# liaoherui/StrainScan

Hardware: AMD Instinct MI355X
Metric: M reads/sec vs 1433-strain E. coli DB (higher is better)
Workload: dtype u64

## Files before the change

### strainscan_amd/csrc/ss_mini.hip

```cpp
#include "ss_common.h"
#include "ss_scan_dev.h"

#include <algorithm>
#include <atomic>
#include <mutex>
#include <type_traits>


namespace {

using namespace ss::dev;

constexpr int MT = 64;
static_assert(MT == 64, "one wave per workgroup: phase 2 compacts with ballots and keeps its counters in scalar registers");
#ifndef SS_Q1CAP
#define SS_Q1CAP 160
#endif
constexpr int Q1CAP = SS_Q1CAP;
static_assert(Q1CAP <= 4096, "q2 keeps a q1b index in 12 bits");
constexpr int Q1CAP_RT = 256;
constexpr int NUM_SGPR = 80;
constexpr int RPL = 2;
constexpr int RPL2 = 1;
constexpr int U3 = 4;
constexpr int MLANES = MT - 2;
constexpr int MTILE = MLANES * PPT;

template <int CAP>
struct QSharedT {
    uint32_t code_[MT + 3];
    uint16_t inv[MT + 2];
    uint32_t q1[CAP + 64];
    alignas(16) uint8_t ib[MT * PPT];
    uint64_t q2[CAP];
    uint32_t cnt[4];
};
template <int CAP>
struct QBloomT {
    uint64_t q1b[CAP];
};

constexpr int COMB_NE = 64;
constexpr int COMB_CH = 4;
constexpr uint32_t COMB_NONE = 0xFFu;
template <int CAP>
struct QCombT {
    static_assert(CAP <= 256, "run indices in bytes");
    uint32_t key[COMB_NE];
    uint32_t nrun[COMB_NE];
    uint32_t acc[COMB_NE][5];
    uint8_t ent[CAP];
    uint8_t list[COMB_NE];
    uint8_t rest[CAP];
};

template <class QS>
__device__ __forceinline__ void kmer_at(const QS &S, uint32_t pos, uint32_t &lo, uint32_t &hi, uint32_t khi_mask = 0x3FFFFFFFu)
{
    const uint32_t w = pos >> 4, sh = 2 * (pos & 15);
    const uint32_t a = S.code_[w + 1], b = S.code_[w + 2], c = S.code_[w + 3];
    lo = __builtin_amdgcn_alignbit(b, a, sh);
    hi = __builtin_amdgcn_alignbit(c, b, sh) & khi_mask;
}

template <class QS>
__device__ __forceinline__ uint32_t mmer_at(const QS &S, uint32_t p)
{
    const uint32_t w = p >> 4;
    return __builtin_amdgcn_alignbit(S.code_[w + 2], S.code_[w + 1], 2 * (p & 15)) & ss::M30;
}
template <class QS>
__device__ __forceinline__ uint32_t win16_at(const QS &S, int32_t p)
{
    const int32_t w = (p >> 4) + 1;
    return __builtin_amdgcn_alignbit(S.code_[w + 1], S.code_[w], 2 * (p & 15));
}

__device__ __forceinline__ uint32_t cand_slot(uint32_t bstart, uint32_t amask, uint32_t q, uint32_t F = 16u)
{
    const uint32_t o = F - q;
    return ((amask >> o) & 1u) ? bstart + 1u + (uint32_t)__popc(amask & ((1u << o) - 1u)) : 0u;
}
__device__ __forceinline__ uint32_t aligned_mask(uint32_t hdr, uint32_t o0, uint32_t F = 16u)
{
    const uint32_t wm = (2u << F) - 1u;
    return ((hdr & wm) << (F - o0)) & wm;
}

template <bool COMB>
__device__ __forceinline__ void count_slot(uint32_t cpos, uint32_t bstart, uint32_t ent, uint32_t *__restrict__ acc5,
                                           uint32_t *__restrict__ counts)
{
    const uint32_t off = cpos - bstart;
    if (COMB && ent != COMB_NONE && off < 20u) atomicAdd(&acc5[ent * 5u + (off >> 2)], 1u << ((off & 3u) * 8u));
    else atomicAdd(&counts[cpos], 1u);
}
template <bool COMB, class QS>
__device__ __forceinline__ void settle_item(const QS &S, uint32_t pos, uint32_t bstart, uint32_t multi, uint32_t cpos,
                                            uint64_t cand, const uint64_t *__restrict__ mkeys,
                                            uint32_t *__restrict__ counts, uint32_t ent = COMB_NONE, uint32_t *__restrict__ acc5 = nullptr,
                                            uint32_t khi_mask = 0x3FFFFFFFu)
{
    uint32_t klo, khi;
    kmer_at(S, pos, klo, khi, khi_mask);
    if ((uint32_t)cand == klo && (uint32_t)(cand >> 32) == khi) {
        count_slot<COMB>(cpos, bstart, ent, acc5, counts);
    } else if (multi) {
        const uint64_t km = ((uint64_t)khi << 32) | klo;
        const uint32_t cnt = (uint32_t)(mkeys[bstart] >> 32);
        for (uint32_t q = 0; q < cnt; q++)
            if (mkeys[bstart + 1 + q] == km) { count_slot<COMB>(bstart + 1 + q, bstart, ent, acc5, counts); break; }
    }
}

__device__ __forceinline__ uint32_t mad24s(uint32_t a, uint32_t b, uint32_t c)
{
    uint32_t d;
    asm("v_mad_u32_u24 %0, %1, %2, %3" : "=v"(d) : "v"(a), "v"(b), "s"(c));
    return d;
}
#define SS_MIN_DPP(i, j) "v_min_u32_dpp %" #i ", %" #j ", %" #i " wave_shl:1 row_mask:0xf bank_mask:0xf bound_ctrl:1\n\t"
__device__ __forceinline__ void min_next_lane8(uint32_t &a0, uint32_t &a1, uint32_t &a2, uint32_t &a3, uint32_t &a4, uint32_t &a5,
                                               uint32_t &a6, uint32_t &a7, uint32_t p0, uint32_t p1, uint32_t p2, uint32_t p3,
                                               uint32_t p4, uint32_t p5, uint32_t p6, uint32_t p7)
{
    asm("s_nop 1\n\t" SS_MIN_DPP(0, 8) SS_MIN_DPP(1, 9) SS_MIN_DPP(2, 10) SS_MIN_DPP(3, 11) SS_MIN_DPP(4, 12) SS_MIN_DPP(5, 13)
        SS_MIN_DPP(6, 14) SS_MIN_DPP(7, 15)
        : "+v"(a0), "+v"(a1), "+v"(a2), "+v"(a3), "+v"(a4), "+v"(a5), "+v"(a6), "+v"(a7)
        : "v"(p0), "v"(p1), "v"(p2), "v"(p3), "v"(p4), "v"(p5), "v"(p6), "v"(p7));
}
__device__ __forceinline__ uint32_t shift_in_ne(uint32_t m, uint32_t a, uint32_t b)
{
    asm("v_cmp_ne_u32 vcc, %1, %2\n\tv_addc_co_u32 %0, vcc, %0, %0, vcc" : "+v"(m) : "v"(a), "v"(b) : "vcc");
    return m;
}

__device__ uint32_t ss_probe_runs[64];

#define SS_MARK(i) asm volatile("; SSMARK " #i)

constexpr int MULTI_MAX = 4;
struct ScanTabs {
    const uint64_t *mkeys[MULTI_MAX];
    const uint4 *pages[MULTI_MAX];
    uint32_t *counts[MULTI_MAX];
    const uint32_t *bloom[MULTI_MAX];
    uint32_t n_pages[MULTI_MAX], cbase[MULTI_MAX], bloom_shift[MULTI_MAX];
    int n;
};

template <int W>
__device__ __forceinline__ void sliding_min(const uint32_t (&x)[32], uint32_t (&out)[PPT])
{
    constexpr int P = W >= 16 ? 16 : W >= 8 ? 8 : W >= 4 ? 4 : 2;
    uint32_t m[32];
#pragma unroll
    for (int i = 0; i < 32; i++) m[i] = x[i];
#pragma unroll
    for (int s2 = 1; s2 < P; s2 <<= 1) {
#pragma unroll
        for (int i = 0; i + s2 < 32; i++) m[i] = min(m[i], m[i + s2]);
    }
#pragma unroll
    for (int j = 0; j < PPT; j++) out[j] = min(m[j], m[j + W - P]);
}

template <int IN, bool BLOOM, bool COMB, int WAVES_PER_SIMD, bool MULTI = false, int KK = 31>
__global__ __launch_bounds__(MT, WAVES_PER_SIMD) __attribute__((amdgpu_num_sgpr(NUM_SGPR))) void scan_mini_kernel(
    const uint8_t *__restrict__ bases, uint64_t n, uint64_t n_tiles, const uint64_t *__restrict__ mkeys0,
    const uint4 *__restrict__ pages0, uint32_t n_pages0, uint32_t *__restrict__ counts0, uint32_t cbase0,
    const uint32_t *__restrict__ bloom, uint32_t bloom_shift, uint32_t xcd_swizzle, const ScanTabs tabs, int k_rt)
{
    static_assert(!(COMB && BLOOM), "a combining scan is for tables that expect hits: they have no use for the minimizer filter");
    static_assert(KK == 31 || KK == 0, "k = 31, or k at run time");
    const uint64_t *__restrict__ mkeys = mkeys0;
    const uint4 *__restrict__ pages = pages0;
    uint32_t *__restrict__ counts = counts0;
    uint32_t n_pages = n_pages0, cbase = cbase0, tab_key = 0u;
    const int K = KK ? KK : k_rt;
    const uint32_t W = (uint32_t)(K - ss::MINI_M + 1), F = W - 1u;
    const uint32_t khi_mask = (1u << (2 * K - 32)) - 1u;
    const uint32_t fmask = F >= 16u ? 0xFFFFFFFFu : (1u << (2u * F)) - 1u;
    static_assert(31 - ss::MINI_M + 1 == PPT + 1, "k = 31: a k-mer window = own m-mers j..15 + neighbour m-mers 0..j");
    constexpr int QC = KK == 31 ? Q1CAP : Q1CAP_RT;
    __shared__ QSharedT<QC> S;
    __shared__ QBloomT<QC> SB;
    __shared__ QCombT<QC> C;
    const int t = threadIdx.x;
    const uint32_t vc1 = ss::MMK_C1;
    constexpr uint64_t CH = COMB ? COMB_CH : 1;

    uint64_t tile = (uint64_t)blockIdx.x * CH, tile_end = n_tiles, stride = gridDim.x, tile0 = 0;
    if (xcd_swizzle & 1u) {
        const uint64_t per = (((n_tiles + 7) >> 3) + CH - 1) / CH * CH, x = blockIdx.x & 7u;
        stride = gridDim.x >> 3;
        tile0 = x * per;
        tile = tile0 + (uint64_t)(blockIdx.x >> 3) * CH;
        tile_end = min(n_tiles, (x + 1) * per);
    }
    auto next_tile = [&](uint64_t tl) -> uint64_t {
        if (CH == 1) return tl + stride;
        return ((tl + 1 - tile0) % CH) ? tl + 1 : tl + 1 + (stride - 1) * CH;
    };
    uint32_t comb_runs = 0;
    if (COMB) {
        C.key[t] = 0u;
        C.nrun[t] = 0u;
#pragma unroll
        for (int w = 0; w < 5; w++) C.acc[t][w] = 0u;
    }
    auto comb_flush = [&]() {
        const uint32_t key = C.key[t];
        const uint64_t occ = __ballot(key != 0u);
        const uint32_t nocc = (uint32_t)__popcll(occ);
        if (key) C.list[__builtin_amdgcn_mbcnt_hi((uint32_t)(occ >> 32), __builtin_amdgcn_mbcnt_lo((uint32_t)occ, 0u))] = (uint8_t)t;
        __syncthreads();
        for (uint32_t g0 = 0; g0 < nocc * 16u; g0 += MT) {
            const uint32_t g = g0 + (uint32_t)t;
            if ((g >> 4) < nocc) {
                const uint32_t e = C.list[g >> 4], off = 1u + (g & 15u);
                const uint32_t c = (C.acc[e][off >> 2] >> ((off & 3u) * 8u)) & 0xFFu;
                if (c) {
                    const uint32_t k1 = C.key[e] - 1u;
                    uint32_t *cb = MULTI ? tabs.counts[k1 >> 30] : counts;
                    atomicAdd(&cb[(k1 & ss::START_MASK) + off], c);
                }
            }
        }
        if (key) {
            const uint32_t w = C.acc[t][4] >> 8;
            if (w) {
                uint32_t *cb = MULTI ? tabs.counts[(key - 1u) >> 30] : counts;
#pragma unroll
                for (uint32_t o = 0; o < 3; o++)
                    if ((w >> (8u * o)) & 0xFFu) atomicAdd(&cb[((key - 1u) & ss::START_MASK) + 17u + o], (w >> (8u * o)) & 0xFFu);
            }
        }
        __syncthreads();
        if (key) {
            C.key[t] = 0u;
            C.nrun[t] = 0u;
#pragma unroll
            for (int w = 0; w < 5; w++) C.acc[t][w] = 0u;
        }
        __syncthreads();
        comb_runs = 0;
    };
    uint32_t wn[4];
    if (tile < tile_end) {
        const uint64_t b0 = tile * MTILE;
        load_in<IN>(bases, b0 + (uint64_t)t * 16, n, wn);
    }
    for (; tile < tile_end; tile = next_tile(tile)) {
        SS_MARK(20);
        {
            uint32_t code, inv;
            decode_in<IN>(wn, code, inv);
            S.code_[t + 1] = code;
            S.inv[t] = (uint16_t)inv;
            if (t == 1) S.cnt[1] = 0;
            const uint64_t nt = next_tile(tile);
            if (nt < tile_end) {
                const uint64_t nb = nt * (uint64_t)MTILE;
                load_in<IN>(bases, nb + (uint64_t)t * 16, n, wn);
            }
        }
        __syncthreads();
        SS_MARK(0);

        uint32_t hm[PPT];
        {
            const uint32_t c0 = S.code_[t + 1], c1 = S.code_[t + 2];
            hm[0] = mad24s(c0, vc1, ss::MMK_C0);
#pragma unroll
            for (int i = 1; i < PPT; i++) hm[i] = mad24s(__builtin_amdgcn_alignbit(c1, c0, 2 * i), vc1, ss::MMK_C0 + (uint32_t)i);
        }
        SS_MARK(1);

        uint32_t live = 0;
        if (KK == 31 && t < MLANES) {
            uint32_t lo;
            __builtin_memcpy(&lo, &S.inv[t], 4);
            uint32_t hi = __builtin_amdgcn_alignbit(S.inv[t + 2], lo, 31);
            lo = __builtin_bitreverse32(lo & 0x7FFFFFFFu);
            lo |= lo << 1; lo |= lo << 2; lo |= lo << 4; lo |= lo << 8; lo |= lo << 16;
            hi |= hi << 1; hi |= hi << 2; hi |= hi << 4; hi |= hi << 8;
            live = ~(__builtin_bitreverse32(lo) | (hi << 1)) & 0xFFFFu;
        } else if (KK != 31 && t < MLANES) {
            uint64_t y = (uint64_t)S.inv[t] | ((uint64_t)S.inv[t + 1] << 16) | ((uint64_t)S.inv[t + 2] << 32);
            y |= y >> 1; y |= y >> 2; y |= y >> 4; y |= y >> 8;
            y |= y >> (K - 16);
            live = ~(uint32_t)y & 0xFFFFu;
        }
        uint32_t need = 0;
        uint32_t mh[PPT];
        if (KK == 31) {
            uint32_t pf[PPT];
            pf[0] = hm[0] + 16u;
#pragma unroll
            for (int j = 1; j < PPT; j++) pf[j] = min(pf[j - 1], hm[j] + 16u);
#pragma unroll
            for (int i = PPT - 2; i >= 0; i--) hm[i] = min(hm[i], hm[i + 1]);
            min_next_lane8(hm[0], hm[1], hm[2], hm[3], hm[4], hm[5], hm[6], hm[7], pf[0], pf[1], pf[2], pf[3], pf[4], pf[5], pf[6], pf[7]);
            min_next_lane8(hm[8], hm[9], hm[10], hm[11], hm[12], hm[13], hm[14], hm[15], pf[8], pf[9], pf[10], pf[11], pf[12], pf[13], pf[14], pf[15]);
#pragma unroll
            for (int j = 0; j < PPT; j++) mh[j] = hm[j];
        } else {
            uint32_t x[32];
#pragma unroll
            for (int i = 0; i < PPT; i++) {
                x[i] = hm[i];
                x[PPT + i] = (uint32_t)__builtin_amdgcn_update_dpp(0, (int)hm[i], 0x130, 0xf, 0xf, false) + 16u;
            }
            switch (W) {
            case 3: sliding_min<3>(x, mh); break;   case 4: sliding_min<4>(x, mh); break;   case 5: sliding_min<5>(x, mh); break;
            case 6: sliding_min<6>(x, mh); break;   case 7: sliding_min<7>(x, mh); break;   case 8: sliding_min<8>(x, mh); break;
            case 9: sliding_min<9>(x, mh); break;   case 10: sliding_min<10>(x, mh); break; case 11: sliding_min<11>(x, mh); break;
            case 12: sliding_min<12>(x, mh); break; case 13: sliding_min<13>(x, mh); break; case 14: sliding_min<14>(x, mh); break;
            case 15: sliding_min<15>(x, mh); break; default: sliding_min<16>(x, mh); break;
            }
        }
        if (live) {
            uint32_t chg = 0u;
#pragma unroll
            for (int j = PPT - 1; j >= 1; j--) chg = shift_in_ne(chg, mh[j], mh[j - 1]);
            chg = (chg << 1) | 1u;
            need = live & (chg | (~live << 1));
            uint32_t pk[4];
#pragma unroll
            for (int w = 0; w < 4; w++) {
                const uint32_t lo = __builtin_amdgcn_perm(mh[4 * w + 1], mh[4 * w], 0x0c0c0400u);
                const uint32_t hi = __builtin_amdgcn_perm(mh[4 * w + 3], mh[4 * w + 2], 0x0c0c0400u);
                pk[w] = __builtin_amdgcn_perm(hi, lo, 0x05040100u);
            }
            reinterpret_cast<uint4 *>(S.ib)[t] = make_uint4(pk[0], pk[1], pk[2], pk[3]);
        }
        SS_MARK(6);
        const uint32_t stop = need | (~live & 0xFFFFu) | 0x10000u;
        uint32_t ext12 = 0;
        {
            const uint32_t first = (uint32_t)__ffs(stop >> 1);
            const uint32_t ownlast = (live >> 15) ? (uint32_t)__clz(need) - 15u : 0u;
            const uint32_t l_mh = (uint32_t)__builtin_amdgcn_update_dpp(0, (int)mh[PPT - 1], 0x138, 0xf, 0xf, false);
            const uint32_t l_own = (uint32_t)__builtin_amdgcn_update_dpp(0, (int)ownlast, 0x138, 0xf, 0xf, false);
            const bool cont = (live & 1u) && l_own && l_mh == mh[0] + 16u && l_own + first <= 16u;
            const uint32_t give = cont ? first << 12 : 0u;
            ext12 = (uint32_t)__builtin_amdgcn_update_dpp(0, (int)give, 0x130, 0xf, 0xf, false);
            if (cont) need &= ~1u;
        }
        uint32_t ovf = 0;
        uint32_t n1;
        {
            const uint32_t mine = (uint32_t)__popc(need);
            const uint32_t incl = wave_inclusive_sum(mine);
            n1 = min((uint32_t)__builtin_amdgcn_readlane((int)incl, 63), (uint32_t)QC);
            const uint32_t mybase = incl - mine;
            if (need) {
                const uint32_t dummy = (uint32_t)QC + (uint32_t)t;
                const uint32_t stop1 = stop >> 1, tbase = (uint32_t)(t * PPT);
                uint32_t idx = mybase;
                for (uint32_t nd = need; nd; idx++) {
                    const uint32_t j = (uint32_t)__ffs(nd) - 1u;
                    nd &= nd - 1u;
                    const uint32_t len = (uint32_t)__ffs(stop1 >> j);
                    S.q1[min(idx, dummy)] = (len << 12) + (tbase + j + (nd ? 0u : ext12));
                }
                if (mybase + mine > (uint32_t)QC) {
                    uint32_t r = mybase;
                    for (uint32_t nd = need; nd; nd &= nd - 1u, r++)
                        if (r >= (uint32_t)QC) ovf |= nd & (0u - nd);
                }
            }
        }
        __syncthreads();
        SS_MARK(2);

        auto run_meta = [&](uint32_t e) {
            const uint32_t rpos = e & 0xFFFu;
            return e | ((((uint32_t)S.ib[rpos] & 31u) - (rpos & 15u)) << 17);
        };
        auto push_found = [&](uint32_t lo, uint32_t mask17, uint32_t meta, uint32_t ridx, bool queued) {
            const uint32_t bstart = lo & ss::START_MASK, multi = lo >> 31;
            const uint32_t amask = aligned_mask(mask17, (meta >> 17) & 31u, F);
            uint32_t i2 = QC;
            if (queued) i2 = atomicAdd(&S.cnt[1], 1u);
            if (i2 < QC) {
                S.q2[i2] = ((uint64_t)(lo & (ss::START_MASK | ss::PG_SOLID)) << 32) | (multi << 31) | (amask << 12) | ridx;
            } else {
                const uint32_t rpos = meta & 0xFFFu, len = (meta >> 12) & 31u;
                for (uint32_t q = 0; q < len; q++) {
                    const uint32_t cpos = cand_slot(bstart, amask, q, F);
                    if (cpos) settle_item<false>(S, rpos + q, bstart, multi, cpos, mkeys[cpos], mkeys, counts, COMB_NONE, nullptr, khi_mask);
                }
            }
        };
        auto scan_page = [&](const uint4 tg, uint32_t page, uint32_t meta, uint32_t h, uint32_t ridx, bool queued) -> bool {
            const uint32_t tt = (h & 0xFFu) * 0x01010101u;
            const uint32_t x0 = tg.x ^ tt, x1 = tg.y ^ tt;
            const uint32_t z0 = ~(((x0 & 0x7F7F7F7Fu) + 0x7F7F7F7Fu) | x0) & 0x80808080u;
            const uint32_t z1 = ~(((x1 & 0x7F7F7F7Fu) + 0x7F7F7F7Fu) | x1) & 0x80808080u;
            uint32_t hit = (z0 >> 7) | (z1 >> 3);
            if (hit) {
                const uint32_t o0 = (meta >> 17) & 31u, len = (meta >> 12) & 31u;
                const char *pb = reinterpret_cast<const char *>(pages) + (uint64_t)page * 64u;
                do {
                    const uint32_t b = (uint32_t)__ffs(hit) - 1u, sl = (b >> 3) + (b & 4u);
                    hit &= hit - 1u;
                    const uint32_t hi8 = (((b & 4u) ? tg.w : tg.z) >> (b & 24u)) & 0xFFu;
                    const bool ref = hi8 & 0x80u;
                    const uint32_t e = hi8 & 31u, j = o0 + e - F;
                    if (ref ? ((hi8 ^ (h >> 8)) & 0x3Fu) == 0u : j < len) {
                        const uint32_t lo = reinterpret_cast<const uint32_t *>(pb + 16)[sl];
                        const uint32_t mid = reinterpret_cast<const uint16_t *>(pb + 48)[sl];
                        if (ref) {
                            push_found(lo, mid | ((hi8 & 0x40u) << 10), meta, ridx, queued);
                        } else if ((mid >> 4) == ((h >> 8) & 0xFFFu)) {
                            const int32_t q = (int32_t)((meta & 0xFFFu) + o0);
                            const uint32_t fa = win16_at(S, q + ss::MINI_M), fb = win16_at(S, q - (int32_t)F);
                            const uint32_t m = ((1u << e) << e) - 1u;
                            if ((((fa & m) | (fb & ~m)) & fmask) == lo) atomicAdd(&counts[cbase + page * 8u + sl], 1u);
                        }
                    }
                } while (hit);
            }
            return (tg.w >> 24) != (uint32_t)ss::PG_EMPTY_HI;
        };
        auto scan_more = [&](uint32_t page, uint32_t meta, uint32_t h, uint32_t ridx, bool queued) {
            uint4 tg;
            do {
                page++;
                tg = pages[(uint64_t)page * 4u];
            } while (scan_page(tg, page, meta, h, ridx, queued));
        };

        SS_MARK(7);
        for (int tb = 0; tb < (MULTI ? tabs.n : 1); tb++) {
        if (MULTI) {
            mkeys = tabs.mkeys[tb]; pages = tabs.pages[tb]; counts = tabs.counts[tb];
            n_pages = tabs.n_pages[tb]; cbase = tabs.cbase[tb]; tab_key = (uint32_t)tb << 30;
            if (BLOOM) { bloom = tabs.bloom[tb]; bloom_shift = tabs.bloom_shift[tb]; }
            if (tb) {
                if (t == 1) S.cnt[1] = 0;
                __syncthreads();
            }
        }
        uint32_t ns = n1;
        if (BLOOM) {
            ns = 0;
            for (uint32_t r0 = 0; r0 < n1; r0 += RPL * MT) {
                SS_MARK(11);
                uint32_t meta[RPL], hs[RPL], bw[RPL];
                bool ok[RPL];
#pragma unroll
                for (int u = 0; u < RPL; u++) {
                    const uint32_t r = r0 + u * MT + t;
                    ok[u] = r < n1;
                    meta[u] = run_meta(S.q1[ok[u] ? r : 0u]);
                    hs[u] = ss::mix30(mmer_at(S, (meta[u] & 0xFFFu) + (meta[u] >> 17)));
                }
#pragma unroll
                for (int u = 0; u < RPL; u++) bw[u] = bloom[hs[u] >> (bloom_shift + 5)];
#pragma unroll
                for (int u = 0; u < RPL; u++) ok[u] = ok[u] && ((bw[u] >> ((hs[u] >> bloom_shift) & 31u)) & 1u);
#pragma unroll
                for (int u = 0; u < RPL; u++) {
                    const uint64_t pass = __ballot(ok[u]);
                    if (ok[u]) SB.q1b[ns + __builtin_amdgcn_mbcnt_hi((uint32_t)(pass >> 32), __builtin_amdgcn_mbcnt_lo((uint32_t)pass, 0u))] =
                        ((uint64_t)hs[u] << 32) | meta[u];
                    ns += (uint32_t)__popcll(pass);
                }
            }
            __syncthreads();
        }
        for (uint32_t i0 = 0; i0 < ns; i0 += RPL2 * MT) {
            SS_MARK(12);
            uint32_t meta[RPL2], hs[RPL2], pgi[RPL2];
            uint4 tg[RPL2];
            bool ok[RPL2];
#pragma unroll
            for (int u = 0; u < RPL2; u++) {
                const uint32_t i = i0 + u * MT + t;
                ok[u] = i < ns;
                if (BLOOM) {
                    const uint64_t sv = SB.q1b[ok[u] ? i : 0u];
                    meta[u] = (uint32_t)sv;
                    hs[u] = (uint32_t)(sv >> 32);
                } else {
                    meta[u] = run_meta(S.q1[ok[u] ? i : 0u]);
                    hs[u] = ss::mix30(mmer_at(S, (meta[u] & 0xFFFu) + (meta[u] >> 17)));
                }
                pgi[u] = ss::page_of(hs[u], n_pages);
                if (ok[u]) tg[u] = pages[(uint64_t)pgi[u] * 4u];
            }
            SS_MARK(13);
#pragma unroll
            for (int u = 0; u < RPL2; u++)
                if (ok[u] && scan_page(tg[u], pgi[u], meta[u], hs[u], i0 + u * MT + t, true)) scan_more(pgi[u], meta[u], hs[u], i0 + u * MT + t, true);
            SS_MARK(14);
        }
        __syncthreads();
        SS_MARK(3);

        {
            const uint32_t n2 = min(S.cnt[1], (uint32_t)QC);
            if (!COMB && (xcd_swizzle & 2u) && t == 0) atomicAdd(&ss_probe_runs[blockIdx.x & 63u], n2);
            bool comb_full = false;
            if (COMB) {
                SS_MARK(10);
                comb_runs += n2;
                for (uint32_t r = (uint32_t)t; r < n2; r += MT) {
                    const uint32_t key = (((uint32_t)(S.q2[r] >> 32) & ss::START_MASK) | tab_key) + 1u;
                    uint32_t i = (key * 0x9E3779B1u) >> 26, e = COMB_NONE;
                    static_assert(COMB_NE == 64, "hash: top six bits");
                    for (int pr = 0; pr < 8; pr++) {
                        const uint32_t old = atomicCAS(&C.key[i], 0u, key);
                        if (old == 0u || old == key) { e = atomicAdd(&C.nrun[i], 1u) < 255u ? i : COMB_NONE; break; }
                        i = (i + 1u) & (COMB_NE - 1u);
                    }
                    C.ent[r] = (uint8_t)e;
                    comb_full = comb_full || e == COMB_NONE;
                }
                comb_full = __ballot(comb_full) != 0ull;
                __syncthreads();
                SS_MARK(9);
            }
            uint32_t n_rest = 0, n_hit = 0;
            auto cand_round = [&](auto UC, uint32_t g0) {
                constexpr int U = decltype(UC)::value;
                SS_MARK(15);
                uint32_t pos[U], bst[U], mul[U], cps[U], ent[U];
                uint64_t cnd[U];
#pragma unroll
                for (int u = 0; u < U; u++) {
                    const uint32_t g = g0 + u * MT + t, q = g & 15u;
                    const bool v = (g >> 4) < n_rest;
                    const uint32_t fi = v ? (COMB ? (uint32_t)C.rest[g >> 4] : (g >> 4)) : 0u;
                    const uint64_t r = S.q2[fi];
                    const uint32_t run = BLOOM ? (uint32_t)SB.q1b[(uint32_t)r & 0xFFFu] : S.q1[(uint32_t)r & 0xFFFu];
                    pos[u] = (run & 0xFFFu) + q;
                    bst[u] = (uint32_t)(r >> 32) & ss::START_MASK;
                    mul[u] = (uint32_t)r >> 31;
                    cps[u] = (v && q < ((run >> 12) & 31u)) ? cand_slot(bst[u], ((uint32_t)r >> 12) & 0x1FFFFu, q, F) : 0u;
                    cnd[u] = mkeys[cps[u]];
                    ent[u] = COMB ? (uint32_t)C.ent[fi] : COMB_NONE;
                }
#pragma unroll
                for (int u = 0; u < U; u++)
                    if (cps[u]) settle_item<COMB>(S, pos[u], bst[u], mul[u], cps[u], cnd[u], mkeys, counts, ent[u], &C.acc[0][0], khi_mask);
                SS_MARK(16);
            };
            if (!COMB) n_rest = n2;
            for (uint32_t r0 = 0; COMB && r0 < n2; r0 += MT) {
                const uint32_t r = r0 + (uint32_t)t;
                const bool v = r < n2;
                const uint64_t q = S.q2[v ? r : 0u];
                const bool solid = v && ((q >> 62) & 1ull);
                uint32_t hitmask = 0;
                const uint64_t om = __ballot(v && !solid);
                if (v && !solid) C.rest[n_rest + __builtin_amdgcn_mbcnt_hi((uint32_t)(om >> 32), __builtin_amdgcn_mbcnt_lo((uint32_t)om, 0u))] = (uint8_t)r;
                n_rest += (uint32_t)__popcll(om);
                if (solid) {
                    const uint32_t bstart = (uint32_t)(q >> 32) & ss::START_MASK, amask = ((uint32_t)q >> 12) & 0x1FFFFu;
                    const uint32_t run = BLOOM ? (uint32_t)SB.q1b[(uint32_t)q & 0xFFFu] : S.q1[(uint32_t)q & 0xFFFu];
                    const uint32_t rpos = run & 0xFFFu, len = (run >> 12) & 31u;
                    const uint32_t am = amask & ~((1u << (W - len)) - 1u);
                    if (am) {
                        const uint32_t o_hi = 31u - (uint32_t)__clz(am), o_lo = (uint32_t)__ffs(am) - 1u, d = o_hi - o_lo;
                        const uint32_t slot_a = bstart + 1u + (uint32_t)__popc(amask & ((1u << o_hi) - 1u));
                        const uint64_t k1 = mkeys[slot_a], k2 = mkeys[slot_a - d];
                        const int32_t P = (int32_t)(rpos + F - o_hi);
                        const uint64_t lo64 = k1 | (k2 << (2u * d));
                        const uint32_t hi32 = d ? (uint32_t)(k2 >> (64u - 2u * d)) : 0u;
                        uint32_t x0 = win16_at(S, P) ^ (uint32_t)lo64;
                        const uint32_t nb1 = d + (uint32_t)K - 16u, nb2 = d + (uint32_t)K > 32u ? d + (uint32_t)K - 32u : 0u;
                        uint32_t x1 = (win16_at(S, P + 16) ^ (uint32_t)(lo64 >> 32)) & (nb1 >= 16u ? 0xFFFFFFFFu : (1u << (2u * nb1)) - 1u);
                        uint32_t x2 = nb2 ? (win16_at(S, P + 32) ^ hi32) & ((1u << (2u * nb2)) - 1u) : 0u;
                        uint32_t match = (2u << d) - 1u;
                        x0 = (x0 | (x0 >> 1)) & 0x55555555u; x1 = (x1 | (x1 >> 1)) & 0x55555555u; x2 = (x2 | (x2 >> 1)) & 0x55555555u;
                        auto strike = [&](uint32_t xb, uint32_t base0) {
                            while (xb) {
                                const uint32_t m = base0 + (((uint32_t)__ffs(xb) - 1u) >> 1);
                                xb &= xb - 1u;
                                const uint32_t hi = min(m, d), lw = m > (uint32_t)K - 1u ? m - ((uint32_t)K - 1u) : 0u;
                                if (lw <= hi) match &= ~(((2u << hi) - 1u) & ~((1u << lw) - 1u));
                            }
                        };
                        strike(x0, 0u); strike(x1, 16u); strike(x2, 32u);
                        if (match) {
                            const uint32_t w_ = 1u;
                            const uint32_t off_a = slot_a - bstart;
                            const uint32_t e_ = COMB ? (uint32_t)C.ent[r] : COMB_NONE;
                            if (COMB && e_ != COMB_NONE && off_a < 20u) {
                                const uint32_t bits = __brev(match) >> (31u - off_a);
#pragma unroll
                                for (uint32_t wd = 0; wd < 5; wd++) {
                                    const uint32_t nib = (bits >> (4u * wd)) & 15u;
                                    if (nib) atomicAdd(&C.acc[e_][wd], ((nib * 0x00204081u) & 0x01010101u) * w_);
                                }
                            } else {
                                hitmask = match;
                                S.q2[r] = ((uint64_t)slot_a << 32) | match;
                            }
                        }
                    }
                }
                const uint64_t hm = __ballot(hitmask != 0u);
                if (hitmask) C.rest[QC - 1u - (n_hit + __builtin_amdgcn_mbcnt_hi((uint32_t)(hm >> 32), __builtin_amdgcn_mbcnt_lo((uint32_t)hm, 0u)))] = (uint8_t)r;
                n_hit += (uint32_t)__popcll(hm);
            }
            if (COMB) __syncthreads();
            for (uint32_t g0 = 0; g0 < n_hit * 16u; g0 += MT) {
                const uint32_t g = g0 + (uint32_t)t;
                if ((g >> 4) < n_hit) {
                    const uint64_t e = S.q2[C.rest[QC - 1u - (g >> 4)]];
                    const uint32_t j = g & 15u, slot_a = (uint32_t)(e >> 32), mt = (uint32_t)e;
                    if ((mt >> j) & 1u) atomicAdd(&counts[slot_a - j], 1u);
                    if (j == 0u && (mt >> 16)) atomicAdd(&counts[slot_a - 16u], 1u);
                }
            }
            const uint32_t total = n_rest * 16u;
            uint32_t g0 = 0;
            for (; g0 < total; g0 += U3 * MT) cand_round(std::integral_constant<int, U3>(), g0);
            if (COMB && comb_full) { __syncthreads(); SS_MARK(4); comb_flush(); SS_MARK(8); }
        }
        if (ovf) {
            for (int j = 0; j < PPT; j++) {
                if (!((ovf >> j) & 1u)) continue;
                const uint32_t len12 = ((uint32_t)__ffs(stop >> (j + 1)) << 12) + ((need >> (j + 1)) ? 0u : ext12);
                const uint32_t meta = run_meta(len12 + (uint32_t)(t * PPT + j));
                const uint32_t h = ss::mix30(mmer_at(S, (meta & 0xFFFu) + (meta >> 17)));
                const uint32_t page = ss::page_of(h, n_pages);
                if (scan_page(pages[(uint64_t)page * 4u], page, meta, h, 0u, false)) scan_more(page, meta, h, 0u, false);
            }
        }
        if (MULTI && tb + 1 < tabs.n) __syncthreads();
        }
        SS_MARK(4);
        __syncthreads();
        SS_MARK(5);
        if (COMB && CH > 1 && comb_runs && ((tile + 1 - tile0) % CH) == 0) { comb_flush(); SS_MARK(8); }
    }
    if (COMB && comb_runs) comb_flush();
}

}

namespace ss {

std::atomic<long long> g_hook_generic_k{0};

constexpr uint64_t PROBE_TILES = 8192;
constexpr double PROBE_RUNS_PER_TILE = 8.0;
static std::mutex probe_mu;

static bool probe_known(ss_db *db, uint64_t set_id, bool *comb)
{
    std::lock_guard<std::mutex> g(probe_mu);
    if (db->probe_set != set_id) return false;
    *comb = db->probe_comb != 0;
    return true;
}

static bool choose_comb(bool flagged, bool binned, bool several, int k, bool verdict)
{
    static const int env = [] { const char *e = getenv("SS_COMBINE"); return e ? atoi(e) : -1; }();
    if (several) return flagged && (env < 0 ? binned : env != 0);
    if (k != 31 || env < 0) return binned && (flagged || (k == 31 && verdict));
    return env == 2 ? binned : (flagged && env != 0);
}

constexpr int scan_mini_waves(bool comb, int kk) { return kk == 0 ? 5 : (comb ? 6 : 8); }

static int launch_scan_mini_pass(ss_db *const *dbs, int n_dbs, bool several, bool bloom, bool comb, bool probe, const uint8_t *b,
                                 uint64_t n, bool packed, hipStream_t stream)
{
    const int k = dbs[0]->k;
    if ((bloom && comb) || (bloom && several && k != 31)) return SS_EINVAL;
    ScanTabs tabs = {};
    for (int i = 0; i < n_dbs; i++) {
        const ss_db *db = dbs[i];
        tabs.mkeys[i] = db->d_mkeys;
        tabs.pages[i] = reinterpret_cast<const uint4 *>(db->d_dir);
        tabs.counts[i] = db->d_counts;
        tabs.n_pages[i] = db->n_dir;
        tabs.cbase[i] = (uint32_t)db->n_mslots;
        tabs.bloom[i] = db->d_bloom;
        tabs.bloom_shift[i] = 30u - db->bloom_bits;
    }
    tabs.n = n_dbs;
    const uint64_t n_tiles = probe ? PROBE_TILES : (n + MTILE - 1) / MTILE;
    const uint64_t units = comb ? (n_tiles + COMB_CH - 1) / COMB_CH : n_tiles;
    unsigned blocks = (unsigned)std::min<uint64_t>(units, (uint64_t)2048 * 256 * (256 / MT));
    blocks = (blocks + 7u) & ~7u;
    const uint32_t swz = 1u | (probe ? 2u : 0u);
    with_input_layout(b, packed, [&](auto in) { with_bool(several, [&](auto multi) { with_bool(k == 31, [&](auto k31) {
        with_bool(bloom, [&](auto bl) { with_bool(comb, [&](auto cb) {
            constexpr int IN = decltype(in)::value, KK = decltype(k31)::value ? 31 : 0;
            constexpr bool MULTI = decltype(multi)::value, BLOOM = decltype(bl)::value, COMB = decltype(cb)::value;
            if constexpr (!(BLOOM && COMB) && !(BLOOM && MULTI && KK == 0))
                hipLaunchKernelGGL((scan_mini_kernel<IN, BLOOM, COMB, scan_mini_waves(COMB, KK), MULTI, KK>), dim3(blocks), dim3(MT), 0,
                                   stream, b, n, n_tiles, tabs.mkeys[0], tabs.pages[0], tabs.n_pages[0], tabs.counts[0], tabs.cbase[0],
                                   tabs.bloom[0], tabs.bloom_shift[0], swz, tabs, k);
        }); });
    }); }); });
    SS_HIP(hipGetLastError());
    return SS_OK;
}

static std::atomic<uint64_t> g_multi_launches[3];

int multi_kind(const ss_db *db)
{
    return db->expect_hits ? MULTI_EXPECT : db->d_bloom ? MULTI_BLOOM : MULTI_PLAIN;
}

constexpr int SHARE_K_MIN = 20;
bool may_share_pass(const ss_db *db)
{
    return db->layout == 1 && db->k >= SHARE_K_MIN && (db->k == 31 || multi_kind(db) != MULTI_BLOOM);
}

int launch_scan_mini_multi(ss_db *const *dbs, int n_dbs, const void *bases_dev, uint64_t n, hipStream_t stream, bool binned, bool packed)
{
    if (n_dbs < 1 || n_dbs > MULTI_MAX || !dbs[0]) return SS_EINVAL;
    const int kind = multi_kind(dbs[0]);
    for (int i = 0; i < n_dbs; i++)
        if (!dbs[i] || !may_share_pass(dbs[i]) || dbs[i]->k != dbs[0]->k || multi_kind(dbs[i]) != kind) return SS_EINVAL;
    const bool comb = choose_comb(kind == MULTI_EXPECT, binned, true, dbs[0]->k, false);
    int rc = launch_scan_mini_pass(dbs, n_dbs, true, kind == MULTI_BLOOM, comb, false, (const uint8_t *)bases_dev, n, packed, stream);
    if (rc) return rc;
    g_multi_launches[kind]++;
    for (int i = 0; i < n_dbs; i++) dbs[i]->launches++;
    return SS_OK;
}

extern "C" int ss_scan_multi_launches(uint64_t out[3])
{
    if (!out) return SS_EINVAL;
    for (int i = 0; i < 3; i++) out[i] = g_multi_launches[i].load();
    return SS_OK;
}

int launch_scan_mini(ss_db *db, const void *bases_dev, uint64_t n, hipStream_t stream, bool binned, uint64_t set_id, bool packed)
{
    const uint8_t *b = (const uint8_t *)bases_dev;
    const long long hk = g_hook_generic_k.load();
    if (db->k == 31 ? (hk == 1 || hk == 2) : (hk != 3 && (hk == 2 || (db->k < SHARE_K_MIN && db->expect_hits))))
        return launch_scan_minik(db, b, n, stream, packed);
    auto comb_if = [&](bool verdict) { return choose_comb(db->expect_hits != 0, binned, false, db->k, verdict); };
    auto pass = [&](bool comb, bool probe) {
        return launch_scan_mini_pass(&db, 1, false, !comb && multi_kind(db) == MULTI_BLOOM, comb, probe, b, n, packed, stream);
    };
    bool verdict = false;
    if (comb_if(false) == comb_if(true)) {}
    else if (set_id && probe_known(db, set_id, &verdict)) {}
    else if ((n + MTILE - 1) / MTILE >= 4 * PROBE_TILES) {
        std::lock_guard<std::mutex> g(probe_mu);
        uint32_t runs[64];
        void *sym = nullptr;
        SS_HIP(hipGetSymbolAddress(&sym, HIP_SYMBOL(ss_probe_runs)));
        SS_HIP(hipMemsetAsync(sym, 0, sizeof(runs), stream));
        int rc = pass(false, true);
        if (rc) return rc;
        SS_HIP(hipMemcpyAsync(runs, sym, sizeof(runs), hipMemcpyDeviceToHost, stream));
        SS_HIP(hipStreamSynchronize(stream));
        uint64_t total = 0;
        for (uint32_t r : runs) total += r;
        db->probe_runs_per_tile = (double)total / (double)PROBE_TILES;
        verdict = db->probe_runs_per_tile >= PROBE_RUNS_PER_TILE;
        db->probe_comb = verdict;
        db->probe_set = set_id;
        b += in_bytes(packed, PROBE_TILES * (uint64_t)MTILE);
        n -= PROBE_TILES * (uint64_t)MTILE;
    }
    return pass(comb_if(verdict), false);
}

}
```

### strainscan_amd/csrc/ss_scan_dev.h

```cpp
#pragma once
#include "ss_common.h"
#include <stdlib.h>
#include <type_traits>

namespace ss {

constexpr int MINI_M = 15;
constexpr uint32_t M30 = 0x3FFFFFFFu;

constexpr uint32_t MMK_C1 = 0x4F1BBu << 5, MMK_C0 = 0x7F4A7C00u;
__host__ __device__ __forceinline__ uint32_t mmkey(uint32_t x)
{
    return (x & 0xFFFFFFu) * MMK_C1 + MMK_C0;
}
constexpr uint32_t KEY_MASK = ~31u;

__host__ __device__ __forceinline__ uint32_t mulhi32(uint32_t a, uint32_t b)
{
#if defined(__HIP_DEVICE_COMPILE__)
    return __umulhi(a, b);
#else
    return (uint32_t)(((uint64_t)a * b) >> 32);
#endif
}
__host__ __device__ __forceinline__ uint32_t mix30(uint32_t x)
{
    uint32_t h = (x * 0x9E3779B1u) & M30;
    h ^= h >> 15;
    h = (h * 0x2C1B3C6Du) & M30;
    h ^= h >> 14;
    return h;
}

constexpr uint32_t HDR_MULTI = 1u << 17;
__host__ __device__ __forceinline__ uint32_t page_of(uint32_t h, uint32_t n_pages) { return mulhi32(h << 2, n_pages); }
constexpr uint32_t PG_SLOTS = 8;
constexpr uint32_t PG_MIN_PAGES = 4096;
constexpr uint8_t PG_EMPTY_TAG = 0xFF, PG_EMPTY_HI = 0x7F;
constexpr uint32_t START_MASK = 0x3FFFFFFFu;
constexpr uint32_t PG_SOLID = 1u << 30;
inline uint32_t choose_inline_max(uint64_t kmers_of_small_minimizers , uint64_t n_distinct)
{
    if (const char *e = getenv("SS_INLINE_MAX")) { const int v = atoi(e); return (uint32_t)(v < 0 ? 0 : v > 8 ? 8 : v); }
    return kmers_of_small_minimizers * 8 < n_distinct ? 0u : 2u;
}
__host__ __device__ __forceinline__ uint32_t flank_of_key(uint64_t key, uint32_t off)
{
    const uint64_t M62 = (1ull << 62) - 1;
    const uint64_t r = off ? (((key >> (2 * off)) | (key << (62 - 2 * off))) & M62) : key;
    return (uint32_t)(r >> 30);
}

constexpr int MINI_K_MIN = MINI_M + 2;
__host__ __device__ __forceinline__ uint32_t flank_of_key_k(uint64_t key, uint32_t off, int k)
{
    const uint64_t M = (1ull << (2 * k)) - 1;
    const uint64_t r = off ? (((key >> (2 * off)) | (key << (2 * k - 2 * off))) & M) : key;
    return (uint32_t)(r >> 30);
}

__host__ __device__ inline uint32_t mini_of_key(uint64_t key, int k, uint32_t *offset)
{
    const int w = k - MINI_M + 1;
    uint32_t best = 0, bo = 0, bx = 0;
    for (int i = 0; i < w; i++) {
        const uint32_t x = (uint32_t)(key >> (2 * i)) & M30;
        const uint32_t h = mmkey(x) & KEY_MASK;
        if (i == 0 || h < best) { best = h; bo = (uint32_t)i; bx = x; }
    }
    *offset = bo;
    return bx;
}

}

namespace ss { namespace dev {

constexpr int SCAN_THREADS = 256;
constexpr int PPT = 16;
constexpr int TILE = SCAN_THREADS * PPT;

__device__ __forceinline__ void encode16(const uint32_t w[4], uint32_t &code, uint32_t &inv)
{
    uint32_t cb[4], fl[4];
#pragma unroll
    for (int d = 0; d < 4; d++) {
        const uint32_t c = (w[d] >> 1) & 0x03030303u;
        const uint32_t letter = __builtin_amdgcn_perm(0u, 0x47544341u, c);
        const uint32_t diff = (w[d] & 0xDFDFDFDFu) ^ letter;
        fl[d] = (((diff & 0x7F7F7F7Fu) + 0x7F7F7F7Fu) | diff) & 0x80808080u;
        cb[d] = __builtin_amdgcn_udot4(c, 0x40100401u, 0u, false);
    }
    code = cb[0] | (cb[1] << 8) | (cb[2] << 16) | (cb[3] << 24);
    const uint32_t lo = __builtin_amdgcn_udot4(fl[1], 0x80402010u, __builtin_amdgcn_udot4(fl[0], 0x08040201u, 0u, false), false);
    const uint32_t hi = __builtin_amdgcn_udot4(fl[3], 0x80402010u, __builtin_amdgcn_udot4(fl[2], 0x08040201u, 0u, false), false);
    inv = (lo | (hi << 8)) >> 7;
}

__device__ __forceinline__ uint32_t newline_mask16(const uint32_t w[4])
{
    uint32_t m = 0;
#pragma unroll
    for (int d = 0; d < 4; d++) {
        const uint32_t x = w[d] ^ 0x0A0A0A0Au;
        const uint32_t z = ~(((x & 0x7F7F7F7Fu) + 0x7F7F7F7Fu) | x) & 0x80808080u;
        m |= __builtin_amdgcn_udot4(z, 0x08040201u, 0u, false) >> 7 << (4 * d);
    }
    return m;
}

template <bool ALIGNED>
__device__ __forceinline__ void load16(const uint8_t *__restrict__ bases, uint64_t off, uint64_t n,
                                       uint32_t w[4])
{
    if (ALIGNED && off + 16 <= n) {
        typedef uint32_t u32x4 __attribute__((ext_vector_type(4)));
        const u32x4 q = __builtin_nontemporal_load(reinterpret_cast<const u32x4 *>(bases + off));
        const uint4 v = make_uint4(q.x, q.y, q.z, q.w);
        w[0] = v.x; w[1] = v.y; w[2] = v.z; w[3] = v.w;
    } else {
#pragma unroll
        for (int d = 0; d < 4; d++) {
            uint32_t x = 0;
#pragma unroll
            for (int b = 0; b < 4; b++) {
                uint64_t p = off + d * 4 + b;
                uint32_t c = (p < n) ? bases[p] : 0x0Au;
                x |= c << (8 * b);
            }
            w[d] = x;
        }
    }
}

enum { IN_ASCII = 0, IN_ASCII_ALIGNED = 1, IN_PACKED = 2 };

template <int IN>
__device__ __forceinline__ void load_in(const uint8_t *__restrict__ bases, uint64_t off, uint64_t n, uint32_t w[4])
{
    if (IN != IN_PACKED) {
        load16<IN == IN_ASCII_ALIGNED>(bases, off, n, w);
    } else if (off + 16 <= n) {
        const uint64_t g6 = (off >> 4) * 6u;
        typedef uint32_t u32x2 __attribute__((ext_vector_type(2)));
        typedef u32x2 u32x2_a4 __attribute__((aligned(4)));
        const u32x2 q = __builtin_nontemporal_load(reinterpret_cast<const u32x2_a4 *>(bases + (g6 & ~3ull)));
        w[0] = q.x; w[1] = q.y; w[2] = (uint32_t)(g6 & 2u) * 0x01010101u;
    } else {
        w[0] = 0x55FF5555u; w[1] = 0x0000FF55u; w[2] = 0u;
    }
}

template <int IN>
__device__ __forceinline__ void decode_in(const uint32_t w[4], uint32_t &code, uint32_t &inv)
{
    if (IN != IN_PACKED) {
        encode16(w, code, inv);
    } else {
        code = __builtin_amdgcn_perm(w[1], w[0], 0x04030100u + w[2]);
        inv = __builtin_amdgcn_perm(w[1], w[0], 0x0C0C0502u + (w[2] & 0xFFFFu));
    }
}

__device__ __forceinline__ uint32_t wave_inclusive_sum(uint32_t v)
{
    v += (uint32_t)__builtin_amdgcn_update_dpp(0, (int)v, 0x111, 0xf, 0xf, false);
    v += (uint32_t)__builtin_amdgcn_update_dpp(0, (int)v, 0x112, 0xf, 0xf, false);
    v += (uint32_t)__builtin_amdgcn_update_dpp(0, (int)v, 0x114, 0xf, 0xf, false);
    v += (uint32_t)__builtin_amdgcn_update_dpp(0, (int)v, 0x118, 0xf, 0xf, false);
    v += (uint32_t)__builtin_amdgcn_update_dpp(0, (int)v, 0x142, 0xa, 0xf, false);
    v += (uint32_t)__builtin_amdgcn_update_dpp(0, (int)v, 0x143, 0xc, 0xf, false);
    return v;
}

__device__ __forceinline__ uint4 packed_letters16(const uint8_t *__restrict__ pk, uint64_t s)
{
    uint32_t t[3];
    __builtin_memcpy(t, pk + (s >> 3) * 3u, 12);
    const uint32_t sh = (uint32_t)s & 7u;
    const uint64_t lo = (uint64_t)t[0] | ((uint64_t)t[1] << 32);
    uint64_t code = (lo & 0xFFFFull) | (((lo >> 24) & 0xFFFFull) << 16) | ((lo >> 48) << 32);
    uint32_t inv = (uint32_t)((lo >> 16) & 0xFFull) | (uint32_t)(((lo >> 40) & 0xFFull) << 8) | ((t[2] & 0xFFu) << 16);
    code >>= 2u * sh;
    inv >>= sh;
    uint32_t w[4];
#pragma unroll
    for (int d = 0; d < 4; d++) {
        uint32_t x = 0;
#pragma unroll
        for (int b = 0; b < 4; b++) {
            const int i = 4 * d + b;
            const uint32_t c = (uint32_t)(code >> (2 * i)) & 3u;
            const uint32_t ch = ((inv >> i) & 1u) ? (uint32_t)'N' : (0x47544341u >> (8u * c)) & 0xFFu;
            x |= ch << (8 * b);
        }
        w[d] = x;
    }
    return make_uint4(w[0], w[1], w[2], w[3]);
}

__host__ __device__ __forceinline__ uint64_t in_bytes(bool packed, uint64_t pos) { return packed ? (pos >> 4) * 6u : pos; }
inline int input_layout(const void *p, bool packed)
{
    return packed ? IN_PACKED : ((((uintptr_t)p) & 15) == 0 ? IN_ASCII_ALIGNED : IN_ASCII);
}
template <class F>
inline void with_input_layout(const void *p, bool packed, F &&f)
{
    switch (input_layout(p, packed)) {
    case IN_PACKED: f(std::integral_constant<int, IN_PACKED>()); break;
    case IN_ASCII_ALIGNED: f(std::integral_constant<int, IN_ASCII_ALIGNED>()); break;
    default: f(std::integral_constant<int, IN_ASCII>()); break;
    }
}
template <class F>
inline void with_bool(bool v, F &&f)
{
    if (v) f(std::true_type()); else f(std::false_type());
}

}}
```

Before: 3224.

## Use 32-bit tile indexing, per-config kernel args, and full-tile fast loads

Switches the scan kernel's tile bookkeeping from 64-bit to 32-bit arithmetic, splitting very large inputs into host-side passes so tile counts fit in 32 bits. Kernel arguments are reduced to a per-configuration struct, so single-table launches no longer carry the multi-table array. Tile loads take a bounds-free fast path for full tiles and a separate path only for the final partial tile. Empty inline asm keeps some values in scalar registers to cut scalar/vector register pressure, at the cost of more code paths and a host loop over passes.

```diff
diff --git a/strainscan_amd/csrc/ss_mini.hip b/strainscan_amd/csrc/ss_mini.hip
--- a/strainscan_amd/csrc/ss_mini.hip
+++ b/strainscan_amd/csrc/ss_mini.hip
@@ -148,6 +148,23 @@
     uint32_t n_pages[MULTI_MAX], cbase[MULTI_MAX], bloom_shift[MULTI_MAX];
     int n;
 };
+struct ScanOne {
+    const uint64_t *mkeys;
+    const uint4 *pages;
+    uint32_t *counts;
+    uint32_t n_pages, cbase;
+};
+struct ScanOneBloom {
+    const uint64_t *mkeys;
+    const uint4 *pages;
+    uint32_t *counts;
+    uint32_t n_pages, cbase;
+    const uint32_t *bloom;
+    uint32_t bloom_shift;
+};
+template <bool MULTI, bool BLOOM>
+using ScanArgT = std::conditional_t<MULTI, ScanTabs, std::conditional_t<BLOOM, ScanOneBloom, ScanOne>>;
+constexpr uint64_t PASS_TILES_MAX = 1ull << 30;
 
 template <int W>
 __device__ __forceinline__ void sliding_min(const uint32_t (&x)[32], uint32_t (&out)[PPT])
@@ -167,16 +184,22 @@
 
 template <int IN, bool BLOOM, bool COMB, int WAVES_PER_SIMD, bool MULTI = false, int KK = 31>
 __global__ __launch_bounds__(MT, WAVES_PER_SIMD) __attribute__((amdgpu_num_sgpr(NUM_SGPR))) void scan_mini_kernel(
-    const uint8_t *__restrict__ bases, uint64_t n, uint64_t n_tiles, const uint64_t *__restrict__ mkeys0,
-    const uint4 *__restrict__ pages0, uint32_t n_pages0, uint32_t *__restrict__ counts0, uint32_t cbase0,
-    const uint32_t *__restrict__ bloom, uint32_t bloom_shift, uint32_t xcd_swizzle, const ScanTabs tabs, int k_rt)
+    const uint8_t *__restrict__ bases, uint32_t n_lo, uint32_t n_full, uint32_t n_tiles, uint32_t xcd_swizzle, int k_rt,
+    const ScanArgT<MULTI, BLOOM> a)
 {
     static_assert(!(COMB && BLOOM), "a combining scan is for tables that expect hits: they have no use for the minimizer filter");
     static_assert(KK == 31 || KK == 0, "k = 31, or k at run time");
-    const uint64_t *__restrict__ mkeys = mkeys0;
-    const uint4 *__restrict__ pages = pages0;
-    uint32_t *__restrict__ counts = counts0;
-    uint32_t n_pages = n_pages0, cbase = cbase0, tab_key = 0u;
+    const uint64_t *__restrict__ mkeys = nullptr;
+    const uint4 *__restrict__ pages = nullptr;
+    uint32_t *__restrict__ counts = nullptr;
+    const uint32_t *__restrict__ bloom = nullptr;
+    uint32_t n_pages = 0u, cbase = 0u, bloom_shift = 0u, tab_key = 0u;
+    if constexpr (!MULTI) {
+        mkeys = a.mkeys; pages = a.pages; counts = a.counts; n_pages = a.n_pages; cbase = a.cbase;
+        if constexpr (BLOOM) { bloom = a.bloom; bloom_shift = a.bloom_shift; }
+    }
+    auto n_tabs = [&]() -> int { if constexpr (MULTI) return a.n; else return 1; };
+    auto counts_of = [&](uint32_t tb) -> uint32_t * { if constexpr (MULTI) return a.counts[tb]; else return counts; };
     const int K = KK ? KK : k_rt;
     const uint32_t W = (uint32_t)(K - ss::MINI_M + 1), F = W - 1u;
     const uint32_t khi_mask = (1u << (2 * K - 32)) - 1u;
@@ -187,20 +210,39 @@
     __shared__ QBloomT<QC> SB;
     __shared__ QCombT<QC> C;
     const int t = threadIdx.x;
+    auto here = [](uint32_t c) -> uint32_t { asm volatile("" : "+s"(c)); return c; };
     const uint32_t vc1 = ss::MMK_C1;
-    constexpr uint64_t CH = COMB ? COMB_CH : 1;
-
-    uint64_t tile = (uint64_t)blockIdx.x * CH, tile_end = n_tiles, stride = gridDim.x, tile0 = 0;
+    constexpr uint32_t CH = COMB ? COMB_CH : 1;
+    constexpr uint32_t TILE_BYTES = MLANES * GROUP_BYTES<IN>;
+
+    uint32_t tile = blockIdx.x * CH, tile_end = n_tiles, stride = gridDim.x, tile0 = 0;
     if (xcd_swizzle & 1u) {
-        const uint64_t per = (((n_tiles + 7) >> 3) + CH - 1) / CH * CH, x = blockIdx.x & 7u;
+        const uint32_t per = (((n_tiles + 7u) >> 3) + CH - 1u) / CH * CH, x = blockIdx.x & 7u;
         stride = gridDim.x >> 3;
         tile0 = x * per;
-        tile = tile0 + (uint64_t)(blockIdx.x >> 3) * CH;
-        tile_end = min(n_tiles, (x + 1) * per);
+        tile = tile0 + (blockIdx.x >> 3) * CH;
+        tile_end = min(n_tiles, (x + 1u) * per);
     }
-    auto next_tile = [&](uint64_t tl) -> uint64_t {
-        if (CH == 1) return tl + stride;
-        return ((tl + 1 - tile0) % CH) ? tl + 1 : tl + 1 + (stride - 1) * CH;
+    const uint32_t stride_probe = stride | ((xcd_swizzle & 2u) << 30);
+    auto next_tile = [&](uint32_t tl) -> uint32_t {
+        const uint32_t st = here(stride_probe) & 0x7FFFFFFFu;
+        if (CH == 1) return tl + st;
+        return ((tl + 1u - tile0) % CH) ? tl + 1u : tl + 1u + (st - 1u) * CH;
+    };
+    const uint32_t lane_off = tile_lane_offset<IN>((uint32_t)t);
+    auto load_tile = [&](uint32_t tl, uint32_t (&w)[4]) {
+        const uint8_t *tile_b = bases + (uint64_t)tl * TILE_BYTES;
+        if (tl < n_full && KK == 0) {
+            const uint32_t g = (uint32_t)t + here(0u);
+            if (IN == IN_PACKED) w[2] = packed_tile_shift(g);
+            load_in_full_tile<IN>(tile_b, tile_lane_offset<IN>(g), w);
+        } else if (tl < n_full) load_in_full_tile<IN>(tile_b, lane_off + here(0u), w);
+        else {
+            const uint32_t g = (uint32_t)t + here(0u);
+            if (IN == IN_PACKED && KK == 0) w[2] = packed_tile_shift(g);
+            load_in_last_tile<IN>(tile_b, g, n_lo - tl * (uint32_t)MTILE, w);
+            asm volatile("; a tile that reaches n");
+        }
     };
     uint32_t comb_runs = 0;
     if (COMB) {
@@ -222,7 +264,7 @@
                 const uint32_t c = (C.acc[e][off >> 2] >> ((off & 3u) * 8u)) & 0xFFu;
                 if (c) {
                     const uint32_t k1 = C.key[e] - 1u;
-                    uint32_t *cb = MULTI ? tabs.counts[k1 >> 30] : counts;
+                    uint32_t *cb = counts_of(k1 >> 30);
                     atomicAdd(&cb[(k1 & ss::START_MASK) + off], c);
                 }
             }
@@ -230,7 +272,7 @@
         if (key) {
             const uint32_t w = C.acc[t][4] >> 8;
             if (w) {
-                uint32_t *cb = MULTI ? tabs.counts[(key - 1u) >> 30] : counts;
+                uint32_t *cb = counts_of((key - 1u) >> 30);
 #pragma unroll
                 for (uint32_t o = 0; o < 3; o++)
                     if ((w >> (8u * o)) & 0xFFu) atomicAdd(&cb[((key - 1u) & ss::START_MASK) + 17u + o], (w >> (8u * o)) & 0xFFu);
@@ -247,10 +289,8 @@
         comb_runs = 0;
     };
     uint32_t wn[4];
-    if (tile < tile_end) {
-        const uint64_t b0 = tile * MTILE;
-        load_in<IN>(bases, b0 + (uint64_t)t * 16, n, wn);
-    }
+    if (IN == IN_PACKED && KK != 0) wn[2] = packed_tile_shift((uint32_t)t);
+    if (tile < tile_end) load_tile(tile, wn);
     for (; tile < tile_end; tile = next_tile(tile)) {
         SS_MARK(20);
         {
@@ -258,12 +298,9 @@
             decode_in<IN>(wn, code, inv);
             S.code_[t + 1] = code;
             S.inv[t] = (uint16_t)inv;
-            if (t == 1) S.cnt[1] = 0;
-            const uint64_t nt = next_tile(tile);
-            if (nt < tile_end) {
-                const uint64_t nb = nt * (uint64_t)MTILE;
-                load_in<IN>(bases, nb + (uint64_t)t * 16, n, wn);
-            }
+            if ((uint32_t)t == here(1u)) S.cnt[1] = 0;
+            const uint32_t nt = next_tile(tile);
+            if (nt < tile_end) load_tile(nt, wn);
         }
         __syncthreads();
         SS_MARK(0);
@@ -278,7 +315,7 @@
         SS_MARK(1);
 
         uint32_t live = 0;
-        if (KK == 31 && t < MLANES) {
+        if (KK == 31 && (uint32_t)t < here(MLANES)) {
             uint32_t lo;
             __builtin_memcpy(&lo, &S.inv[t], 4);
             uint32_t hi = __builtin_amdgcn_alignbit(S.inv[t + 2], lo, 31);
@@ -434,11 +471,11 @@
         };
 
         SS_MARK(7);
-        for (int tb = 0; tb < (MULTI ? tabs.n : 1); tb++) {
-        if (MULTI) {
-            mkeys = tabs.mkeys[tb]; pages = tabs.pages[tb]; counts = tabs.counts[tb];
-            n_pages = tabs.n_pages[tb]; cbase = tabs.cbase[tb]; tab_key = (uint32_t)tb << 30;
-            if (BLOOM) { bloom = tabs.bloom[tb]; bloom_shift = tabs.bloom_shift[tb]; }
+        for (int tb = 0; tb < n_tabs(); tb++) {
+        if constexpr (MULTI) {
+            mkeys = a.mkeys[tb]; pages = a.pages[tb]; counts = a.counts[tb];
+            n_pages = a.n_pages[tb]; cbase = a.cbase[tb]; tab_key = (uint32_t)tb << 30;
+            if (BLOOM) { bloom = a.bloom[tb]; bloom_shift = a.bloom_shift[tb]; }
             if (tb) {
                 if (t == 1) S.cnt[1] = 0;
                 __syncthreads();
@@ -503,7 +540,9 @@
 
         {
             const uint32_t n2 = min(S.cnt[1], (uint32_t)QC);
-            if (!COMB && (xcd_swizzle & 2u) && t == 0) atomicAdd(&ss_probe_runs[blockIdx.x & 63u], n2);
+            if (!COMB && (here(stride_probe) >> 31)) {
+                if ((uint32_t)t == here(0u)) atomicAdd(&ss_probe_runs[here(blockIdx.x) & 63u], n2);
+            }
             bool comb_full = false;
             if (COMB) {
                 SS_MARK(10);
@@ -633,7 +672,7 @@
                 if (scan_page(pages[(uint64_t)page * 4u], page, meta, h, 0u, false)) scan_more(page, meta, h, 0u, false);
             }
         }
-        if (MULTI && tb + 1 < tabs.n) __syncthreads();
+        if (MULTI && tb + 1 < n_tabs()) __syncthreads();
         }
         SS_MARK(4);
         __syncthreads();
@@ -688,7 +727,11 @@
         tabs.bloom_shift[i] = 30u - db->bloom_bits;
     }
     tabs.n = n_dbs;
-    const uint64_t n_tiles = probe ? PROBE_TILES : (n + MTILE - 1) / MTILE;
+    const uint64_t all_tiles = probe ? PROBE_TILES : (n + MTILE - 1) / MTILE;
+    for (uint64_t first = 0; first < all_tiles; first += PASS_TILES_MAX) {
+    const uint64_t n_tiles = std::min<uint64_t>(all_tiles - first, PASS_TILES_MAX);
+    if (first) { b += in_bytes(packed, PASS_TILES_MAX * (uint64_t)MTILE); n -= PASS_TILES_MAX * (uint64_t)MTILE; }
+    const uint64_t n_full = std::min<uint64_t>(n_tiles, n >= (uint64_t)MT * PPT ? (n - (uint64_t)MT * PPT) / MTILE + 1 : 0);
     const uint64_t units = comb ? (n_tiles + COMB_CH - 1) / COMB_CH : n_tiles;
     unsigned blocks = (unsigned)std::min<uint64_t>(units, (uint64_t)2048 * 256 * (256 / MT));
     blocks = (blocks + 7u) & ~7u;
@@ -697,13 +740,22 @@
         with_bool(bloom, [&](auto bl) { with_bool(comb, [&](auto cb) {
             constexpr int IN = decltype(in)::value, KK = decltype(k31)::value ? 31 : 0;
             constexpr bool MULTI = decltype(multi)::value, BLOOM = decltype(bl)::value, COMB = decltype(cb)::value;
-            if constexpr (!(BLOOM && COMB) && !(BLOOM && MULTI && KK == 0))
+            if constexpr (!(BLOOM && COMB) && !(BLOOM && MULTI && KK == 0)) {
+                ScanArgT<MULTI, BLOOM> a;
+                if constexpr (MULTI) {
+                    a = tabs;
+                } else {
+                    a.mkeys = tabs.mkeys[0]; a.pages = tabs.pages[0]; a.counts = tabs.counts[0];
+                    a.n_pages = tabs.n_pages[0]; a.cbase = tabs.cbase[0];
+                    if constexpr (BLOOM) { a.bloom = tabs.bloom[0]; a.bloom_shift = tabs.bloom_shift[0]; }
+                }
                 hipLaunchKernelGGL((scan_mini_kernel<IN, BLOOM, COMB, scan_mini_waves(COMB, KK), MULTI, KK>), dim3(blocks), dim3(MT), 0,
-                                   stream, b, n, n_tiles, tabs.mkeys[0], tabs.pages[0], tabs.n_pages[0], tabs.counts[0], tabs.cbase[0],
-                                   tabs.bloom[0], tabs.bloom_shift[0], swz, tabs, k);
+                                   stream, b, (uint32_t)n, (uint32_t)n_full, (uint32_t)n_tiles, swz, k, a);
+            }
         }); });
     }); }); });
     SS_HIP(hipGetLastError());
+    }
     return SS_OK;
 }
 
diff --git a/strainscan_amd/csrc/ss_scan_dev.h b/strainscan_amd/csrc/ss_scan_dev.h
--- a/strainscan_amd/csrc/ss_scan_dev.h
+++ b/strainscan_amd/csrc/ss_scan_dev.h
@@ -148,6 +148,59 @@
         w[0] = q.x; w[1] = q.y; w[2] = (uint32_t)(g6 & 2u) * 0x01010101u;
     } else {
         w[0] = 0x55FF5555u; w[1] = 0x0000FF55u; w[2] = 0u;
+    }
+}
+
+template <int IN>
+constexpr uint32_t GROUP_BYTES = IN == IN_PACKED ? 6u : 16u;
+
+template <int IN>
+__device__ __forceinline__ uint32_t tile_lane_offset(uint32_t g) { return IN == IN_PACKED ? (g * 6u) & ~3u : g * 16u; }
+__device__ __forceinline__ uint32_t packed_tile_shift(uint32_t g) { return ((g * 6u) & 2u) ? 0x02020202u : 0u; }
+template <int IN>
+__device__ __forceinline__ void load_in_full_tile(const uint8_t *__restrict__ tile_b, uint32_t lane_off, uint32_t w[4])
+{
+    if (IN == IN_PACKED) {
+        typedef uint32_t u32x2 __attribute__((ext_vector_type(2)));
+        typedef u32x2 u32x2_a4 __attribute__((aligned(4)));
+        const u32x2 q = __builtin_nontemporal_load(reinterpret_cast<const u32x2_a4 *>(tile_b + lane_off));
+        w[0] = q.x; w[1] = q.y;
+    } else if (IN == IN_ASCII_ALIGNED) {
+        typedef uint32_t u32x4 __attribute__((ext_vector_type(4)));
+        const u32x4 q = __builtin_nontemporal_load(reinterpret_cast<const u32x4 *>(tile_b + lane_off));
+        w[0] = q.x; w[1] = q.y; w[2] = q.z; w[3] = q.w;
+    } else {
+#pragma unroll
+        for (int d = 0; d < 4; d++) {
+            uint32_t x = 0;
+#pragma unroll
+            for (int b = 0; b < 4; b++) x |= (uint32_t)tile_b[lane_off + (uint32_t)(d * 4 + b)] << (8 * b);
+            w[d] = x;
+        }
+    }
+}
+
+template <int IN>
+__device__ __forceinline__ void load_in_last_tile(const uint8_t *__restrict__ tile_b, uint32_t g, uint32_t rem, uint32_t w[4])
+{
+    if (IN == IN_PACKED) {
+        if (g * 16u + 16u <= rem) {
+            load_in_full_tile<IN>(tile_b, tile_lane_offset<IN>(g), w);
+        } else {
+            const bool s2 = (g * 6u) & 2u;
+            w[0] = s2 ? 0x55550000u : 0x55FF5555u; w[1] = s2 ? 0xFF5555FFu : 0x0000FF55u;
+        }
+    } else {
+#pragma unroll
+        for (int d = 0; d < 4; d++) {
+            uint32_t x = 0;
+#pragma unroll
+            for (int b = 0; b < 4; b++) {
+                const uint32_t p = g * 16u + d * 4 + b;
+                x |= (p < rem ? (uint32_t)tile_b[p] : 0x0Au) << (8 * b);
+            }
+            w[d] = x;
+        }
     }
 }
 
```

Result: no change. 3239 (median of 6 runs) (+0.5%).
